# 18281818221/kalle-audio

Hardware: AMD Instinct MI355X
Metric: audio-seconds/sec (node) DiT train step, 10s@12.5Hz x1024 latents (higher is better)
Workload: dtype bf16; 1 GPU; DiT train step (fwd+bwd+allreduce+Adam), 24 blocks D=1536 h=24, 10 s @ 12.5 Hz x 1024 latents (T=125+1 prepend), S=130 x 768 cross-attn cond; DiT shape chosen by this build (reference defines none); global_batch=256, per_gpu_batch=256, parallelism=dp1, objective=v, io_channels=1024, global_cond_type=prepend

## Files before the change

### include/kalle_hip.h

```cpp
#ifndef KALLE_HIP_H
#define KALLE_HIP_H
#include <stdint.h>

#ifdef __cplusplus
extern "C" {
#endif

#define KALLE_BF16 0
#define KALLE_F32 1

int kalle_abi_version(void);
const char* kalle_target_arch(void);
const char* kalle_last_error(void);

typedef struct kalle_gemm_epilogue {
    const float* bias;
    const float* gate;
    int64_t ldg;
    int32_t rows_per_batch;
    const float* residual;
    int64_t ldr;
    int32_t accumulate;
    float alpha;
    int32_t c_rows_per_batch;
// ... 204 lines not shown
typedef struct kalle_opt_ctl {
    float   norm;
    float   coef;
    int32_t nonfinite;
    int32_t skip;
    int64_t skipped;
    int64_t clipped;
} kalle_opt_ctl;
int kalle_grad_norm_ws_bytes(int nslots);
int kalle_grad_sumsq(const float* grad, int64_t n, void* ws, int slot, int nslots, void* stream);
int kalle_grad_norm_finish(const void* ws, int nslots, float grad_scale, float max_norm, int skip_nonfinite,
                           kalle_opt_ctl* ctl, void* stream);
int kalle_adam_step_ctl(float* param, const float* grad, float* exp_avg, float* exp_avg_sq, void* param_bf16,
                        int64_t n, float lr, float beta1, float beta2, float eps, float weight_decay, int decoupled,
                        int step, float grad_scale, const kalle_opt_ctl* ctl, void* stream);

int kalle_weight_norm_fold(const float* v, const float* g, float* w_packed, int d0, int d1, int ksize,
                           int transposed, void* stream);
typedef struct kalle_act {
    int32_t code;
    int32_t logscale;
    const float* alpha;
    const float* beta;
    float param;
} kalle_act;
typedef struct kalle_conv_epilogue {
    const void* residual;
    float out_scale;
    int32_t accumulate;
    int32_t tanh;
// ... 159 lines not shown
```

### kalle_audio_amd/build.py

```python
import os
import subprocess
import sys
from concurrent.futures import ThreadPoolExecutor

HERE = os.path.dirname(os.path.abspath(__file__))
CSRC = os.path.join(HERE, "csrc")
OUT = os.path.join(HERE, "libkalle_hip.so")
SOURCES = ["gemm.hip", "gemm2.hip", "norm.hip", "elementwise.hip", "attention.hip", "conv1d.hip", "conv1d_bwd.hip",
           "llasa.hip", "conformer.hip"]
FLAGS = ["-O3", "--offload-arch=gfx950", "-fPIC", "-std=c++17", "-ffast-math", "-fno-finite-math-only",
         "-Wno-unused-value"]


def source_stamp():
    import hashlib
    h = hashlib.sha256()
    files = sorted(os.path.join(CSRC, f) for f in os.listdir(CSRC) if f.endswith((".hip", ".h")))
    files.append(os.path.join(HERE, "..", "include", "kalle_hip.h"))
    for f in files:
        h.update(os.path.basename(f).encode())
        h.update(open(f, "rb").read())
    return h.hexdigest()[:16]


def _needs(obj, deps):
    if not os.path.exists(obj):
        return True
    t = os.path.getmtime(obj)
    return any(os.path.getmtime(d) > t for d in deps)


def build(verbose=True, force=False, extra_flags=(), out=None, objdir_name="build", only=None):
    global OUT
    hipcc = os.environ.get("HIPCC", "/opt/rocm/bin/hipcc")
    objdir = os.path.join(HERE, objdir_name)
    out = out or OUT
    os.makedirs(objdir, exist_ok=True)
    hdrs = [os.path.join(CSRC, "common.h"), os.path.join(CSRC, "gemm_common.h"), os.path.join(HERE, "..", "include", "kalle_hip.h")]
    srcs = [s for s in SOURCES if os.path.exists(os.path.join(CSRC, s))]
    jobs = []
    for s in srcs:
        src = os.path.join(CSRC, s)
        obj = os.path.join(objdir, s.replace(".hip", ".o"))
        if force or _needs(obj, [src] + hdrs):
            jobs.append([hipcc] + FLAGS + list(extra_flags) + ["-c", src, "-o", obj])

    def run(cmd):
        if verbose:
            print(" ".join(cmd), flush=True)
        r = subprocess.run(cmd, capture_output=True, text=True)
        if r.returncode != 0:
            raise RuntimeError("hipcc failed:\n" + r.stdout + r.stderr)
        if verbose and r.stderr.strip():
# ... 18 lines not shown
```

### kalle_audio_amd/csrc/elementwise.hip

```cpp
#include <stdio.h>
#include <stdlib.h>

#include "common.h"
#include "../../include/kalle_hip.h"

namespace {

inline int grid_for(int64_t work_items, int block) {
    int64_t g = (work_items + block - 1) / block;
    if (g > 2048) g = 2048;
    if (g < 1) g = 1;
    return (int)g;
}

__global__ __launch_bounds__(256) void swiglu_fwd_kernel(const bf16_t* __restrict__ h, bf16_t* __restrict__ out,
                                                         int64_t rows, int inner) {
    const int cpr = inner >> 3;
    const int64_t total = rows * cpr;
    for (int64_t i = (int64_t)blockIdx.x * blockDim.x + threadIdx.x; i < total; i += (int64_t)gridDim.x * blockDim.x) {
        const int64_t r = i / cpr;
        const int c = (int)(i - r * cpr) * 8;
        const i32x4 xv = *reinterpret_cast<const i32x4*>(h + r * 2 * inner + c);
        const i32x4 gv = *reinterpret_cast<const i32x4*>(h + r * 2 * inner + inner + c);
        i32x4 o;
// ... 306 lines not shown
    const float wj = w[j];
    for (int b = 0; b < nbatch; ++b) {
        const float k = 6.283185307179586f * t[b];
        const float f = k * wj;
        acc += k * (dout[(int64_t)b * 2 * half + half + j] * cosf(f) - dout[(int64_t)b * 2 * half + j] * sinf(f));
    }
    dw[j] = acc;
}

__device__ __forceinline__ void adam_body(float* __restrict__ p, const float* __restrict__ g,
                                          float* __restrict__ m, float* __restrict__ v,
                                          bf16_t* __restrict__ pb, int64_t n, float lr, float b1, float b2,
                                          float eps, float wd, int decoupled, float bc1, float bc2,
                                          float gscale, const int64_t first, const int64_t stride) {
    const int64_t n4 = n >> 2;
    for (int64_t i = first; i < n4; i += stride) {
        f32x4 pv = reinterpret_cast<f32x4*>(p)[i];
        const f32x4 gv = reinterpret_cast<const f32x4*>(g)[i];
        f32x4 mv = reinterpret_cast<f32x4*>(m)[i];
        f32x4 vv = reinterpret_cast<f32x4*>(v)[i];
#pragma unroll
        for (int e = 0; e < 4; ++e) {
            float gr = gv[e] * gscale;
            if (decoupled) pv[e] *= (1.f - lr * wd); else gr += wd * pv[e];
            mv[e] = b1 * mv[e] + (1.f - b1) * gr;
            vv[e] = b2 * vv[e] + (1.f - b2) * gr * gr;
            const float denom = sqrtf(vv[e]) / bc2 + eps;
            pv[e] -= (lr / bc1) * (mv[e] / denom);
        }
        reinterpret_cast<f32x4*>(p)[i] = pv;
        reinterpret_cast<f32x4*>(m)[i] = mv;
        reinterpret_cast<f32x4*>(v)[i] = vv;
        if (pb) {
            i32x2 o;
            o[0] = (int)pack_bf16x2(pv[0], pv[1]);
            o[1] = (int)pack_bf16x2(pv[2], pv[3]);
            reinterpret_cast<i32x2*>(pb)[i] = o;
        }
    }
    if (blockIdx.x == 0 && threadIdx.x < (n & 3)) {
        const int64_t i = (n4 << 2) + threadIdx.x;
        float pv = p[i], gr = g[i] * gscale, mv = m[i], vv = v[i];
        if (decoupled) pv *= (1.f - lr * wd); else gr += wd * pv;
        mv = b1 * mv + (1.f - b1) * gr;
        vv = b2 * vv + (1.f - b2) * gr * gr;
        pv -= (lr / bc1) * (mv / (sqrtf(vv) / bc2 + eps));
        p[i] = pv; m[i] = mv; v[i] = vv;
        if (pb) pb[i] = f32_to_bf16(pv);
    }
}

__global__ __launch_bounds__(256) void adam_kernel(float* __restrict__ p, const float* __restrict__ g,
                                                   float* __restrict__ m, float* __restrict__ v,
                                                   bf16_t* __restrict__ pb, int64_t n, float lr, float b1, float b2,
                                                   float eps, float wd, int decoupled, float bc1, float bc2,
                                                   float gscale) {
    adam_body(p, g, m, v, pb, n, lr, b1, b2, eps, wd, decoupled, bc1, bc2, gscale,
              (int64_t)blockIdx.x * blockDim.x + threadIdx.x, (int64_t)gridDim.x * blockDim.x);
}

__global__ __launch_bounds__(256) void adam_ctl_kernel(float* __restrict__ p, const float* __restrict__ g,
                                                       float* __restrict__ m, float* __restrict__ v,
                                                       bf16_t* __restrict__ pb, int64_t n, float lr, float b1, float b2,
                                                       float eps, float wd, int decoupled, float bc1, float bc2,
                                                       float gscale, const kalle_opt_ctl* __restrict__ ctl) {
    if (ctl->skip) return;
    adam_body(p, g, m, v, pb, n, lr, b1, b2, eps, wd, decoupled, bc1, bc2, gscale * ctl->coef,
              (int64_t)blockIdx.x * blockDim.x + threadIdx.x, (int64_t)gridDim.x * blockDim.x);
}

__device__ __forceinline__ void sumsq_acc(const f32x4 x, double& acc, uint32_t& bad) {
#pragma unroll
    for (int e = 0; e < 4; ++e) {
        const float xe = x[e];
        const double d = (double)xe;
        acc += d * d;
        bad |= (uint32_t)((__builtin_bit_cast(uint32_t, xe) & 0x7f800000u) == 0x7f800000u);
    }
}

__global__ __launch_bounds__(KALLE_GRAD_NORM_BLOCK) void grad_sumsq_kernel(const float* __restrict__ g, int64_t n,
                                                                           double* __restrict__ part,
                                                                           int32_t* __restrict__ flag) {
// ... 225 lines not shown
}

extern "C" int kalle_adam_step_ctl(float* param, const float* grad, float* exp_avg, float* exp_avg_sq, void* param_bf16,
                                   int64_t n, float lr, float beta1, float beta2, float eps, float weight_decay,
                                   int decoupled, int step, float grad_scale, const kalle_opt_ctl* ctl, void* stream) {
    if (!param || !grad || !exp_avg || !exp_avg_sq || !ctl || n <= 0 || step <= 0) return KALLE_ERR_ARG;
    if ((uintptr_t)ctl & 7) return KALLE_ERR_ARG;
    const float bc1 = 1.f - powf(beta1, (float)step);
    const float bc2 = sqrtf(1.f - powf(beta2, (float)step));
    const int agrid = (int)std::min<int64_t>(((n >> 2) + 255) / 256 + 1, 16384);
    KALLE_LAUNCH(adam_ctl_kernel, dim3(agrid), dim3(256), 0, static_cast<hipStream_t>(stream), param,
                       grad, exp_avg, exp_avg_sq, static_cast<bf16_t*>(param_bf16), n, lr, beta1, beta2, eps,
                       weight_decay, decoupled, bc1, bc2, grad_scale, ctl);
    return kalle_check_launch();
}
extern "C" int kalle_grad_norm_ws_bytes(int nslots) {
    if (nslots <= 0 || nslots > (1 << 16)) return KALLE_ERR_ARG;
    return nslots * KALLE_GRAD_NORM_SLOT_BYTES;
}
extern "C" int kalle_grad_sumsq(const float* grad, int64_t n, void* ws, int slot, int nslots, void* stream) {
    if (!grad || !ws || n <= 0 || nslots <= 0 || nslots > (1 << 16) || slot < 0 || slot >= nslots) return KALLE_ERR_ARG;
    if (((uintptr_t)grad & 15) || ((uintptr_t)ws & 15)) return KALLE_ERR_ARG;
    char* base = static_cast<char*>(ws) + (int64_t)slot * KALLE_GRAD_NORM_SLOT_BYTES;
    KALLE_LAUNCH(grad_sumsq_kernel, dim3(KALLE_GRAD_NORM_PARTIALS), dim3(KALLE_GRAD_NORM_BLOCK), 0,
                 static_cast<hipStream_t>(stream), grad, n, reinterpret_cast<double*>(base),
                 reinterpret_cast<int32_t*>(base + KALLE_GRAD_NORM_PARTIALS * 8));
    return kalle_check_launch();
}
extern "C" int kalle_grad_norm_finish(const void* ws, int nslots, float grad_scale, float max_norm, int skip_nonfinite,
                                      kalle_opt_ctl* ctl, void* stream) {
// ... 45 lines not shown
```

### kalle_audio_amd/csrc/gemm2.hip

```cpp
#include <stdio.h>
#include <stdlib.h>
#include <string.h>

#include <algorithm>
#include <functional>
#include <type_traits>
#include <utility>

#include "gemm_common.h"
#include "../../include/kalle_hip.h"

namespace {

constexpr int BK2 = 64;
#define GPTR(p) ((const __attribute__((address_space(1))) void*)(p))

__device__ __attribute__((aligned(64))) const unsigned kalle_zero_block[16] = {0, 0, 0, 0, 0, 0, 0, 0, 0, 0, 0, 0, 0, 0, 0, 0};

template <bool KM, int R, int NW>
struct Loader {
    static constexpr int PER_WAVE = (R / 8) / NW;
    const bf16_t* src[PER_WAVE];
    int64_t kstep;

// ... 667 lines not shown
    hipDeviceProp_t prop;
    v = hipGetDeviceProperties(&prop, dev) == hipSuccess && prop.multiProcessorCount > 0 ? prop.multiProcessorCount : 256;
    v &= ~7;
    if (v < 8) v = 8;
    cached[dev & 63].store(v, std::memory_order_relaxed);
    return v;
}

#define MFMA32(FA, FB)                                                                                         \
    _Pragma("unroll") for (int mt = 0; mt < 8; ++mt) _Pragma("unroll") for (int nt = 0; nt < 4; ++nt)          \
        acc[mt][nt] = __builtin_amdgcn_mfma_f32_16x16x32_bf16(__builtin_bit_cast(bf16x8, FA[mt]),              \
                                                              __builtin_bit_cast(bf16x8, FB[nt]), acc[mt][nt], 0, 0, 0)

constexpr int SCHED_SETS = 256;
constexpr int SCHED_LINE = 32;
__device__ int kalle_gemm_sched[SCHED_SETS][9 * SCHED_LINE];

__device__ __forceinline__ int sched_issue(int* sched, int xcd) { return atomicAdd(sched + xcd * SCHED_LINE, 1); }
__device__ __forceinline__ int sched_resolve(int xcd, int raw, int first_round, int ntiles) {
    const int id = xcd + 8 * (first_round + raw);
    return id < ntiles ? id : ntiles;
}
__device__ __forceinline__ void sched_leave(int* sched, int nwg) {
    if (atomicAdd(sched + 8 * SCHED_LINE, 1) == nwg - 1) {
#pragma unroll
        for (int i = 0; i < 9; ++i) atomicExch(sched + i * SCHED_LINE, 0);
    }
}

template <bool A_KM, bool B_KM, bool C_F32, int GLU, bool XCD_RASTER, bool PERSIST>
__device__ __forceinline__ void gemm3_tiles(const GemmParams& p, int tile0, int tstride, int tile_end, int ntiles_raster, int kt0,
                                            int nk) {
    const int kvalid = p.K % BK2;
    const int tail_t = kvalid ? (p.K + BK2 - 1) / BK2 - 1 - kt0 : -1;
    constexpr int WN = 4, TM = 8, NW = 8;
    constexpr int BM = 256, BN = 256;
    constexpr int A_BYTES = BM * 128, B_BYTES = BN * 128, STAGE = A_BYTES + B_BYTES;
    extern __shared__ __attribute__((aligned(16))) char smem[];
    const unsigned lds0 = (unsigned)(size_t)LDS_PTR(char, smem);

    const int tid = threadIdx.x, lane = tid & 63;
// ... 143 lines not shown
                if (nk > 1) {
                    la.issue_at(smem + s_last, wave, lane, 1, tail_t, kvalid);
                    lb.issue_at(smem + s_last + A_BYTES, wave, lane, 1, tail_t, kvalid);
                }
                if (sched && tid == 0) drawn = sched_issue(sched, blockIdx.x & 7);
            }
        };
        wave_epilogue<C_F32, TM, GLU>(p, acc, smem + 2 * STAGE, wave, lane, m0 + arow, GLU == 1 ? tn * 128 + wn * 32 : n0 + bcol,
                                      hook, tile);
        prefetched = has_next;
        s0 = s_last ^ STAGE;
        if constexpr (!PERSIST) break;
    }
}

template <bool A_KM, bool B_KM, bool C_F32, int GLU = 0>
__global__ __launch_bounds__(512, 2) void gemm3_kernel(GemmParams p) {
    const int nk_all = (p.K + BK2 - 1) / BK2;
    const int ntiles = p.tiles_m * p.tiles_n;
    if constexpr (A_KM) {
        if (p.mix_na >= 0) {
            const int na = p.mix_na, sa = p.mix_sa;
            int bid = blockIdx.x, tile, slice, per;
            if (bid < na * sa) { tile = bid % na; slice = bid / na; per = (nk_all + sa - 1) / sa; }
            else { bid -= na * sa; const int nb = ntiles - na; tile = na + bid % nb; slice = bid / nb; per = (nk_all + sa) / (sa + 1); }
            const int kt0 = slice * per, nk = min(per, nk_all - kt0);
            if (nk <= 0) return;
            gemm3_tiles<A_KM, B_KM, C_F32, GLU, true, false>(p, tile, 0, tile + 1, ntiles, kt0, nk);
        } else {
            const int kt0 = blockIdx.y * p.ktiles_per_split;
            gemm3_tiles<A_KM, B_KM, C_F32, GLU, true, false>(p, blockIdx.x, 0, blockIdx.x + 1, ntiles, kt0,
                                                             min(p.ktiles_per_split, nk_all - kt0));
        }
    } else {
        gemm3_tiles<A_KM, B_KM, C_F32, GLU, true, true>(p, blockIdx.x, gridDim.x, ntiles, ntiles, 0, nk_all);
        if (p.sched_set > 0 && threadIdx.x == 0) sched_leave(&kalle_gemm_sched[p.sched_set - 1][0], gridDim.x);
    }
}

struct GroupProblem {
    const bf16_t* A;
    const bf16_t* B;
    float* C;
    int64_t lda, ldb, ldc;
    int M, N, K;
    int tiles_m, tiles_n, group_m;
    int unsplit, splits;
    int r1_start, r2_start;
};
struct GroupParams {
// ... 43 lines not shown
    p.alpha = 1.f;
    p.rows_per_batch = 1;
    p.accumulate = gp.overwrite ? 0 : 1;
    p.atomic = whole ? 0 : 1;
    const int ntiles = q.tiles_m * q.tiles_n, nk_all = (q.K + BK2 - 1) / BK2;
    p.tiles_m = q.tiles_m; p.tiles_n = q.tiles_n; p.group_m = q.group_m;
    int kt0 = 0, nk = nk_all;
    if (!whole) {
        const int per = (nk_all + q.splits - 1) / q.splits;
        kt0 = slice * per;
        nk = min(per, nk_all - kt0);
        if (nk <= 0) return;
    }
    gemm3_tiles<true, true, true, 0, false, false>(p, tile, 0, tile + 1, ntiles, kt0, nk);
}

template <bool A_KM, bool B_KM, bool C_F32, int GLU = 0>
int launch3(const GemmParams& p, hipStream_t st) {
    constexpr int lds = GEMM3_LDS;
    static std::atomic<uint64_t> lds_ok{0};
    kalle_allow_lds(reinterpret_cast<const void*>(gemm3_kernel<A_KM, B_KM, C_F32, GLU>), lds, lds_ok);
    dim3 grid(p.tiles_m * p.tiles_n, p.splits), block(512);
    if (p.mix_na >= 0) {
        const int ntiles = p.tiles_m * p.tiles_n;
        grid = dim3(p.mix_na * p.mix_sa + (ntiles - p.mix_na) * (p.mix_sa + 1), 1);
    } else if (!A_KM) {
        if (p.splits != 1) return KALLE_ERR_UNSUPPORTED;
        const int cus = kalle_cu_count();
        if ((int)grid.x > cus) {
            GemmParams q = p;
            grid.x = cus;
            static std::atomic<unsigned> next_set{0};
            hipStreamCaptureStatus cap = hipStreamCaptureStatusNone;
            const bool capturing = hipStreamIsCapturing(st, &cap) == hipSuccess && cap != hipStreamCaptureStatusNone;
            q.sched_set = !capturing ? 1 + (int)(next_set.fetch_add(1, std::memory_order_relaxed) % SCHED_SETS) : 0;
            KALLE_LAUNCH((gemm3_kernel<A_KM, B_KM, C_F32, GLU>), grid, block, lds, st, q);
            return kalle_check_launch();
        }
    }
    KALLE_LAUNCH((gemm3_kernel<A_KM, B_KM, C_F32, GLU>), grid, block, lds, st, p);
    return kalle_check_launch();
}

int launch3_layout(const GemmParams& p, bool a_km, bool b_km, bool f32, hipStream_t st) {
    if (!a_km && !b_km) return f32 ? launch3<false, false, true>(p, st) : launch3<false, false, false>(p, st);
    if (!a_km && b_km) return f32 ? launch3<false, true, true>(p, st) : launch3<false, true, false>(p, st);
    if (a_km && b_km) return launch3<true, true, true>(p, st);
    return KALLE_ERR_UNSUPPORTED;
}

// ... 348 lines not shown

namespace {
__global__ __launch_bounds__(256) void hold_cus_kernel(int ticks) {
    extern __shared__ char hold_smem[];
    if (ticks < 0) hold_smem[threadIdx.x] = 1;
    const unsigned long long t_end = __builtin_amdgcn_s_memrealtime() + (unsigned long long)ticks;
    while (__builtin_amdgcn_s_memrealtime() < t_end) __builtin_amdgcn_s_sleep(64);
}
}
extern "C" int kalle_debug_hold_cus(int nwg, int lds_bytes, int microseconds, void* stream) {
    if (nwg <= 0 || nwg > 4096 || lds_bytes < 0 || lds_bytes > 65536 || microseconds < 0 || microseconds > 1000000) return KALLE_ERR_ARG;
    KALLE_LAUNCH(hold_cus_kernel, dim3(nwg), dim3(256), lds_bytes, static_cast<hipStream_t>(stream), microseconds * 100);
    return kalle_check_launch();
}

static thread_local int g_last_plan = 0;
extern "C" int kalle_gemm_last_plan(void) { return g_last_plan; }

extern "C" int kalle_gemm_plan(const void* A, int64_t lda, int a_kmajor, const void* B, int64_t ldb, int b_kmajor,
                               void* C, int64_t ldc, int c_dtype, int M, int N, int K,
                               const kalle_gemm_epilogue* ep, int* plan) {
    if (!plan) return KALLE_ERR_ARG;
    GemmParams p; GemmPlan g;
    const int rc = plan_gemm(A, lda, a_kmajor, B, ldb, b_kmajor, C, ldc, c_dtype, M, N, K, ep, false, p, g);
    if (rc == KALLE_OK) *plan = g.word;
    return rc;
}

extern "C" int kalle_gemm_bf16(const void* A, int64_t lda, int a_kmajor, const void* B, int64_t ldb, int b_kmajor,
                               void* C, int64_t ldc, int c_dtype, int M, int N, int K,
// ... 145 lines not shown
```

### kalle_audio_amd/csrc/gemm_common.h

```cpp
#pragma once
#include "common.h"

struct GemmParams {
    const bf16_t* A;
    const bf16_t* B;
    void* C;
    int64_t lda, ldb, ldc;
    int M, N, K;
    const float* bias;
    const float* gate;
    int64_t ldg;
    int rows_per_batch;
    const float* residual;
    int64_t ldr;
    int accumulate;
    int tiles_n;
    float alpha;
    int c_rpb, c_brows, c_roff;
    const uint8_t* row_mask;
    int tiles_m, splits, ktiles_per_split, atomic, group_m, tile_n;
    int mix_na, mix_sa;
    int glu_mode, glu_inner;
    void* glu_aux;
    float* glu_dbias;
    int64_t slab_stride;
    unsigned long long* stamps;
    int sched_set;
};

__device__ __forceinline__ void gemm_tile_coords(int bid, int nwg, int tiles_m, int tiles_n, int gm, int& tm, int& tn) {
    const int qd = nwg >> 3, rm = nwg & 7, xcd = bid & 7;
    const int wg = (xcd < rm ? xcd * (qd + 1) : rm * (qd + 1) + (xcd - rm) * qd) + (bid >> 3);
    const int per_group = gm * tiles_n;
    const int group = wg / per_group;
    const int first_m = group * gm;
    const int gsz = min(gm, tiles_m - first_m);
    const int in = wg - group * per_group;
    tm = first_m + in % gsz;
    tn = in / gsz;
}

__device__ __forceinline__ int xcd_contiguous(int bid, int nwg) {
// ... 66 lines not shown
```

### kalle_audio_amd/engine.py

```python
import math
import contextlib
import os

import torch
import torch.distributed as dist

from . import ops


class FusedAdam(torch.optim.Optimizer):

    def __init__(self, params, lr=1e-3, betas=(0.9, 0.999), eps=1e-8, weight_decay=0.0, adam_w_mode=True):
        super().__init__(params, dict(lr=lr, betas=betas, eps=eps, weight_decay=weight_decay, adam_w_mode=adam_w_mode))

    @torch.no_grad()
    def step(self, closure=None):
        loss = closure() if closure is not None else None
        for g in self.param_groups:
            for p in g["params"]:
                if p.grad is None:
                    continue
                st = self.state[p]
                if not st:
                    st["step"] = 0
# ... 167 lines not shown
            self._norm_ws = ops.grad_norm_ws(len(self._norm_slot), device)
            self._ctl = ops.OptCtl(device)
        self.shard_opt = (os.environ.get("KALLE_SHARD_OPTIMIZER", "0") == "1" and comm_dtype == torch.float32
                          and self.world & (self.world - 1) == 0 and self.world <= 64)
        self._shard_bufs = {}
        self.overlap_adam = device.type == "cuda" and os.environ.get("KALLE_OVERLAP_ADAM", "1") != "0"
        side = self.overlap_adam or (device.type == "cuda" and self.shard_opt)
        self._opt_stream = torch.cuda.Stream(device=device) if side else None
        self._comm_stream = torch.cuda.Stream(device=device) if side else None
        self._comm_events = 0
        self._shard_ev = None
        self._opt_done = set()
        self._opt_lr = None
        self._overlap_now = False
        self.overlap_min_rows = int(os.environ.get("KALLE_OVERLAP_ADAM_MIN_ROWS", "4096"))
        for n, blk in self.blocks:
            pre = n + "."
            blk._kalle_grad_sinks = {k[len(pre):]: self.flat.grad_view(k) for k in self.flat.names if k.startswith(pre)}
            blk._kalle_grad_accumulate = False
            blk._kalle_bucket_key = pre if pre in self.flat.bucket_range else None
            blk._kalle_on_backward_done = self._on_block_done
        for (na, a), (nb, b_) in zip(self.blocks, self.blocks[1:]):
            if (isinstance(a, TransformerBlock) and isinstance(b_, TransformerBlock) and na.rsplit(".", 1)[0] == nb.rsplit(".", 1)[0]
                    and getattr(b_, "layer_ix", -1) == getattr(a, "layer_ix", -9) + 1):
                object.__setattr__(b_, "_kalle_prev_block", a)
        for n, p in named:
            if getattr(p, "_kalle_wants_sink", False) and bucket_of(n) == "_rest":
                p._kalle_grad_sink = self.flat.grad_view(n)

    def _comm_active(self):
# ... 146 lines not shown

    def _on_block_done(self, blk):
        key = blk._kalle_bucket_key
        if key is None or not self._boundary():
            return
        if self._sharded_active():
            ev = None
            if self.flat.grad.is_cuda:
                ev = torch.cuda.Event()
                ev.record(torch.cuda.current_stream())
            self._sharded_bucket(key, ev)
            return
        if not self._overlap_now:
            self._allreduce(self.flat.bucket_grad(key))
            return
        ev = torch.cuda.Event()
        ev.record(torch.cuda.current_stream())
        self._queue_bucket([key], ev)

    def _begin_optimizer_step(self):
        k = self.step_count + 1
        self._opt_lr = self.lr * (self.lr_schedule(k - 1) if self.lr_schedule else 1.0)
        self._opt_done = set()
        self._norm_done = set()
        self._norm_final = False
        self._comm_events = 0
        self._shard_ev = None

    def _adam_bucket(self, key):
        a, b = self.flat.bucket_range[key]
        self._adam_range(a, b)
        self._opt_done.add(key)

    def _adam_range(self, a, b, grad=None):
        if b <= a:
            return
        f = self.flat
        ops.adam_step(f.param[a:b], f.grad[a:b] if grad is None else grad, self.exp_avg[a:b], self.exp_avg_sq[a:b],
                      f.param_bf16[a:b] if f.param_bf16 is not None else None, lr=self._opt_lr, beta1=self.betas[0],
                      beta2=self.betas[1], eps=self.eps, weight_decay=self.weight_decay, decoupled=self.decoupled,
                      step=self.step_count + 1, grad_scale=1.0 / (self.world * self.grad_accum_steps))

    def _boundary(self):
        return (self.micro + 1) % self.grad_accum_steps == 0

    def _finish_comm(self):
        if self._overlap_now and self._boundary():
            cur = torch.cuda.current_stream()
            ev = torch.cuda.Event()
            ev.record(cur)
            done = self._norm_done if self._norm_gate else self._opt_done
            self._queue_bucket([k for k in self.flat.bucket_keys if k not in done], ev)
            if self._norm_on:
                with torch.cuda.stream(self._opt_stream):
                    self._norm_finish()
                    if self._norm_gate:
                        self._adam_ctl_all()
            timed = self.comm_timing is not None
            if timed:
                e0, e1 = torch.cuda.Event(enable_timing=True), torch.cuda.Event(enable_timing=True)
                e0.record()
# ... 47 lines not shown
        if first:
            if clear_once:
                self.flat.grad.zero_()
            else:
                if grouped:
                    for _, blk in self.blocks:
                        a, b = self.flat.small_range.get(blk._kalle_bucket_key, (0, 0))
                        if b > a:
                            self.flat.grad[a:b].zero_()
                for key in ("_rest", "_vae"):
                    if key in self.flat.bucket_range:
                        self.flat.bucket_grad(key).zero_()
        if self._boundary():
            self._begin_optimizer_step()
            self._overlap_now = self.overlap_adam and (rows >= self.overlap_min_rows or not self.blocks)
        loss.backward()
        self._finish_comm()
        if self._boundary():
            self.optimizer_step()
        self.micro += 1

    def enable_ema(self, **kw):
        self.ema_schedule = EMASchedule(**kw)
        self.ema = self.flat.param.clone()
        return self

    def _ema_update(self):
        d = self.ema_schedule.next()
        if d is None:
            return
# ... 92 lines not shown
```

### kalle_audio_amd/ops.py

```python
import ctypes
import os

import torch

from . import _lib
from ._lib import KALLE_BF16, KALLE_F32, GemmEpilogue, check


def _stream():
    return ctypes.c_void_p(torch.cuda.current_stream().cuda_stream)


def _dt(t):
    if t.dtype == torch.bfloat16:
        return KALLE_BF16
    if t.dtype == torch.float32:
        return KALLE_F32
    raise TypeError(f"unsupported dtype {t.dtype}")


def _p(t):
    if t is None:
        return None
    if not t.is_cuda:
# ... 359 lines not shown


WEIGHTS_EPOCH = 0


def adam_step(param, grad, exp_avg, exp_avg_sq, param_bf16, *, lr, beta1=0.9, beta2=0.999, eps=1e-8, weight_decay=0.0,
              decoupled=False, step=1, grad_scale=1.0):
    global WEIGHTS_EPOCH
    WEIGHTS_EPOCH += 1
    lib = _lib.load()
    check(lib.kalle_adam_step(_p(param), _p(grad), _p(exp_avg), _p(exp_avg_sq), _p(param_bf16), param.numel(), lr,
                              beta1, beta2, eps, weight_decay, int(decoupled), step, grad_scale, _stream()),
          "kalle_adam_step")


GRAD_NORM_PARTIALS = 1024
GRAD_NORM_BLOCK = 256
GRAD_NORM_UNROLL = 4


class OptCtl:

    def __init__(self, device):
        self.t = torch.zeros(8, device=device, dtype=torch.int32)
        self.norm = self.t[0:1].view(torch.float32)
        self.coef = self.t[1:2].view(torch.float32)
        self.nonfinite = self.t[2:3]
        self.skip = self.t[3:4]
        self.skipped = self.t[4:6].view(torch.int64)
        self.clipped = self.t[6:8].view(torch.int64)
# ... 638 lines not shown
```

Baseline: 11740 audio-seconds/sec.

## Run Adam bucket updates in GEMM tail workgroups via a device job ring

Adds a device-side ring of Adam jobs. During backward, each finished gradient bucket is appended to the ring instead of being queued on a separate optimizer stream. GEMM kernels get a variant that pulls Adam chunks from the ring, presumably in idle tail workgroups, and a flush kernel finishes any remaining chunks at the step boundary. The Adam math is also rewritten with FMAs and reciprocal approximations, and the ring path can use nontemporal loads and stores. The aim is to hide optimizer memory traffic under GEMM tails, at the cost of added atomics, extra GEMM register and LDS pressure, and slightly different rounding in Adam.

```diff
diff --git a/include/kalle_hip.h b/include/kalle_hip.h
--- a/include/kalle_hip.h
+++ b/include/kalle_hip.h
@@ -242,6 +242,20 @@
 int kalle_adam_step_ctl(float* param, const float* grad, float* exp_avg, float* exp_avg_sq, void* param_bf16,
                         int64_t n, float lr, float beta1, float beta2, float eps, float weight_decay, int decoupled,
                         int step, float grad_scale, const kalle_opt_ctl* ctl, void* stream);
+
+#define KALLE_ADAM_RING_JOBS 32
+#define KALLE_ADAM_CHUNK_FLOAT4 2048
+#define KALLE_ADAM_RING_QUERY_INTS (4 + 2 * KALLE_ADAM_RING_JOBS)
+int kalle_adam_ring_create(void** ring);
+int kalle_adam_ring_destroy(void* ring);
+int kalle_adam_ring_append(void* ring, float* param, const float* grad, float* exp_avg, float* exp_avg_sq, void* param_bf16,
+                           int64_t n, float lr, float beta1, float beta2, float eps, float weight_decay, int decoupled,
+                           int step, float grad_scale, int chunk_float4, void* stream);
+int kalle_adam_ring_pending(void* ring);
+int kalle_gemm_attach_adam_ring(void* ring);
+int kalle_adam_flush(void* ring, void* stream);
+int kalle_adam_ring_query(void* ring, int64_t* out, void* stream);
+int kalle_debug_adam_chunks(void* ring, int nwg, int threads, int lds_bytes, int take, void* stream);
 
 int kalle_weight_norm_fold(const float* v, const float* g, float* w_packed, int d0, int d1, int ksize,
                            int transposed, void* stream);
diff --git a/kalle_audio_amd/build.py b/kalle_audio_amd/build.py
--- a/kalle_audio_amd/build.py
+++ b/kalle_audio_amd/build.py
@@ -36,7 +36,8 @@
     objdir = os.path.join(HERE, objdir_name)
     out = out or OUT
     os.makedirs(objdir, exist_ok=True)
-    hdrs = [os.path.join(CSRC, "common.h"), os.path.join(CSRC, "gemm_common.h"), os.path.join(HERE, "..", "include", "kalle_hip.h")]
+    hdrs = [os.path.join(CSRC, "common.h"), os.path.join(CSRC, "gemm_common.h"), os.path.join(CSRC, "adam_tails.h"),
+            os.path.join(HERE, "..", "include", "kalle_hip.h")]
     srcs = [s for s in SOURCES if os.path.exists(os.path.join(CSRC, s))]
     jobs = []
     for s in srcs:
diff --git a/kalle_audio_amd/csrc/adam_tails.h b/kalle_audio_amd/csrc/adam_tails.h
--- /dev/null
+++ b/kalle_audio_amd/csrc/adam_tails.h
@@ -0,0 +1,157 @@
+#pragma once
+#include "common.h"
+
+constexpr int ADAM_RING_JOBS = 32;
+
+struct AdamScalars {
+    float lr, b1, b2, eps, wd, bc1, bc2, gscale;
+    int decoupled;
+};
+
+struct alignas(128) AdamJob {
+    float* p;
+    const float* g;
+    float* m;
+    float* v;
+    bf16_t* pb;
+    int64_t n;
+    AdamScalars s;
+    int chunk4;
+    int nt;
+    int nchunks;
+    alignas(128) int cursor;
+};
+
+struct alignas(128) AdamRing {
+    int njobs;
+    alignas(128) int head;
+    alignas(128) int64_t chunks_tails;
+    int64_t chunks_all;
+    AdamJob job[ADAM_RING_JOBS];
+};
+
+struct KalleAdamRing {
+    AdamRing* dev;
+    int njobs;
+};
+
+struct AdamConsts {
+    float wd, b1, b2, eps, gscale, lr, bc1;
+    float decay;
+    float inv_bc2;
+    int decoupled;
+};
+__device__ __forceinline__ AdamConsts adam_consts(float lr, float b1, float b2, float eps, float wd, int decoupled, float bc1,
+                                                  float bc2, float gscale) {
+    AdamConsts c;
+    c.wd = wd; c.b1 = b1; c.b2 = b2; c.eps = eps; c.gscale = gscale; c.lr = lr; c.bc1 = bc1;
+    c.decay = __builtin_fmaf(-lr, wd, 1.f);
+    c.inv_bc2 = __builtin_amdgcn_rcpf(bc2);
+    c.decoupled = decoupled;
+    return c;
+}
+__device__ __forceinline__ void adam_update(float& p, const float g, float& m, float& v, const AdamConsts& c) {
+#pragma clang fp reassociate(off) contract(off)
+    const float gs = g * c.gscale;
+    const float gr = c.decoupled ? gs : __builtin_fmaf(p, c.wd, gs);
+    const float pd = c.decoupled ? p * c.decay : p;
+    const float g2 = gr * gr;
+    v = __builtin_fmaf(__builtin_fmaf(-gr, gr, v), c.b2, g2);
+    m = __builtin_fmaf(m - gr, c.b1, gr);
+    const float denom = __builtin_fmaf(__builtin_amdgcn_sqrtf(v), c.inv_bc2, c.eps);
+    p = __builtin_fmaf(-(c.lr * m), __builtin_amdgcn_rcpf(c.bc1 * denom), pd);
+}
+__device__ __forceinline__ void adam_update4(f32x4& pv, const f32x4 gv, f32x4& mv, f32x4& vv, const AdamConsts& c) {
+#pragma unroll
+    for (int e = 0; e < 4; ++e) {
+        float p = pv[e], m = mv[e], v = vv[e];
+        adam_update(p, gv[e], m, v, c);
+        pv[e] = p; mv[e] = m; vv[e] = v;
+    }
+}
+__device__ __forceinline__ void adam_update1(float* __restrict__ p, const float* __restrict__ g, float* __restrict__ m,
+                                             float* __restrict__ v, bf16_t* __restrict__ pb, int64_t i, const AdamConsts& c) {
+    float pv = p[i], mv = m[i], vv = v[i];
+    adam_update(pv, g[i], mv, vv, c);
+    p[i] = pv; m[i] = mv; v[i] = vv;
+    if (pb) pb[i] = f32_to_bf16(pv);
+}
+
+constexpr int ADAM_CHUNK_UNROLL = 4;
+template <bool NT>
+__device__ __forceinline__ void adam_chunk(const AdamJob& job, int c) {
+    float* __restrict__ p = job.p;
+    const float* __restrict__ g = job.g;
+    float* __restrict__ m = job.m;
+    float* __restrict__ v = job.v;
+    bf16_t* __restrict__ pb = job.pb;
+    const AdamScalars s = job.s;
+    const AdamConsts k = adam_consts(s.lr, s.b1, s.b2, s.eps, s.wd, s.decoupled, s.bc1, s.bc2, s.gscale);
+    const int64_t n4 = job.n >> 2;
+    const int64_t begin = (int64_t)c * job.chunk4;
+    const int64_t end = min(begin + (int64_t)job.chunk4, n4);
+    const int nt = blockDim.x;
+    auto ld = [](const float* base, int64_t i) {
+        const f32x4* q = reinterpret_cast<const f32x4*>(base) + i;
+        return NT ? __builtin_nontemporal_load(q) : *q;
+    };
+    auto st = [](float* base, int64_t i, const f32x4 x) {
+        f32x4* q = reinterpret_cast<f32x4*>(base) + i;
+        if (NT) __builtin_nontemporal_store(x, q); else *q = x;
+    };
+    for (int64_t i0 = begin + threadIdx.x; i0 < end; i0 += (int64_t)ADAM_CHUNK_UNROLL * nt) {
+        f32x4 pv[ADAM_CHUNK_UNROLL], gv[ADAM_CHUNK_UNROLL], mv[ADAM_CHUNK_UNROLL], vv[ADAM_CHUNK_UNROLL];
+#pragma unroll
+        for (int u = 0; u < ADAM_CHUNK_UNROLL; ++u) {
+            const int64_t i = i0 + (int64_t)u * nt;
+            if (i < end) { pv[u] = ld(p, i); gv[u] = ld(g, i); mv[u] = ld(m, i); vv[u] = ld(v, i); }
+        }
+#pragma unroll
+        for (int u = 0; u < ADAM_CHUNK_UNROLL; ++u) {
+            const int64_t i = i0 + (int64_t)u * nt;
+            if (i < end) {
+                adam_update4(pv[u], gv[u], mv[u], vv[u], k);
+                st(p, i, pv[u]); st(m, i, mv[u]); st(v, i, vv[u]);
+                if (pb) {
+                    i32x2 o;
+                    o[0] = (int)pack_bf16x2(pv[u][0], pv[u][1]);
+                    o[1] = (int)pack_bf16x2(pv[u][2], pv[u][3]);
+                    i32x2* q = reinterpret_cast<i32x2*>(pb) + i;
+                    if (NT) __builtin_nontemporal_store(o, q); else *q = o;
+                }
+            }
+        }
+    }
+    if (c == job.nchunks - 1 && (int)threadIdx.x < (int)(job.n & 3))
+        adam_update1(p, g, m, v, pb, (n4 << 2) + threadIdx.x, k);
+}
+
+__device__ __forceinline__ void adam_chunks(AdamRing* ring, volatile int* box, int* stop, int stop_at, int take) {
+    int j = 0, njobs = 0;
+    if (threadIdx.x == 0) {
+        njobs = min(__hip_atomic_load(&ring->njobs, __ATOMIC_RELAXED, __HIP_MEMORY_SCOPE_AGENT), ADAM_RING_JOBS);
+        j = njobs > 0 ? min(atomicAdd(&ring->head, 0), njobs) : 0;
+    }
+    for (int it = 0;; it ^= 2) {
+        if (threadIdx.x == 0) {
+            int c = -1;
+            if (!stop || atomicAdd(stop, 0) < stop_at) {
+                while (j < njobs) {
+                    c = atomicAdd(&ring->job[j].cursor, take);
+                    if (c < ring->job[j].nchunks) break;
+                    c = -1;
+                    atomicMax(&ring->head, ++j);
+                }
+            }
+            box[it] = j;
+            box[it + 1] = c;
+        }
+        __syncthreads();
+        const int jj = box[it], c = box[it + 1];
+        if (c < 0) break;
+        const AdamJob& job = ring->job[jj];
+        const int cend = min(c + take, job.nchunks);
+        if (job.nt) { for (int k = c; k < cend; ++k) adam_chunk<true>(job, k); }
+        else { for (int k = c; k < cend; ++k) adam_chunk<false>(job, k); }
+    }
+}
diff --git a/kalle_audio_amd/csrc/elementwise.hip b/kalle_audio_amd/csrc/elementwise.hip
--- a/kalle_audio_amd/csrc/elementwise.hip
+++ b/kalle_audio_amd/csrc/elementwise.hip
@@ -2,6 +2,7 @@
 #include <stdlib.h>
 
 #include "common.h"
+#include "adam_tails.h"
 #include "../../include/kalle_hip.h"
 
 namespace {
@@ -344,20 +345,13 @@
                                           float eps, float wd, int decoupled, float bc1, float bc2,
                                           float gscale, const int64_t first, const int64_t stride) {
     const int64_t n4 = n >> 2;
+    const AdamConsts k = adam_consts(lr, b1, b2, eps, wd, decoupled, bc1, bc2, gscale);
     for (int64_t i = first; i < n4; i += stride) {
         f32x4 pv = reinterpret_cast<f32x4*>(p)[i];
         const f32x4 gv = reinterpret_cast<const f32x4*>(g)[i];
         f32x4 mv = reinterpret_cast<f32x4*>(m)[i];
         f32x4 vv = reinterpret_cast<f32x4*>(v)[i];
-#pragma unroll
-        for (int e = 0; e < 4; ++e) {
-            float gr = gv[e] * gscale;
-            if (decoupled) pv[e] *= (1.f - lr * wd); else gr += wd * pv[e];
-            mv[e] = b1 * mv[e] + (1.f - b1) * gr;
-            vv[e] = b2 * vv[e] + (1.f - b2) * gr * gr;
-            const float denom = sqrtf(vv[e]) / bc2 + eps;
-            pv[e] -= (lr / bc1) * (mv[e] / denom);
-        }
+        adam_update4(pv, gv, mv, vv, k);
         reinterpret_cast<f32x4*>(p)[i] = pv;
         reinterpret_cast<f32x4*>(m)[i] = mv;
         reinterpret_cast<f32x4*>(v)[i] = vv;
@@ -369,14 +363,7 @@
         }
     }
     if (blockIdx.x == 0 && threadIdx.x < (n & 3)) {
-        const int64_t i = (n4 << 2) + threadIdx.x;
-        float pv = p[i], gr = g[i] * gscale, mv = m[i], vv = v[i];
-        if (decoupled) pv *= (1.f - lr * wd); else gr += wd * pv;
-        mv = b1 * mv + (1.f - b1) * gr;
-        vv = b2 * vv + (1.f - b2) * gr * gr;
-        pv -= (lr / bc1) * (mv / (sqrtf(vv) / bc2 + eps));
-        p[i] = pv; m[i] = mv; v[i] = vv;
-        if (pb) pb[i] = f32_to_bf16(pv);
+        adam_update1(p, g, m, v, pb, (n4 << 2) + threadIdx.x, k);
     }
 }
 
@@ -397,6 +384,37 @@
     if (ctl->skip) return;
     adam_body(p, g, m, v, pb, n, lr, b1, b2, eps, wd, decoupled, bc1, bc2, gscale * ctl->coef,
               (int64_t)blockIdx.x * blockDim.x + threadIdx.x, (int64_t)gridDim.x * blockDim.x);
+}
+
+__global__ void adam_ring_append_kernel(AdamRing* ring, AdamJob job) {
+    const int j = ring->njobs;
+    if (j >= ADAM_RING_JOBS) return;
+    job.cursor = 0;
+    ring->job[j] = job;
+    __threadfence();
+    ring->njobs = j + 1;
+}
+__global__ void adam_ring_account_kernel(AdamRing* ring) {
+    int64_t took = 0, all = 0;
+    for (int j = 0; j < ring->njobs; ++j) {
+        took += min(atomicAdd(&ring->job[j].cursor, 0), ring->job[j].nchunks);
+        all += ring->job[j].nchunks;
+    }
+    ring->chunks_tails += took;
+    ring->chunks_all += all;
+}
+constexpr int ADAM_FLUSH_TAKE = 4, ADAM_FLUSH_GRID = 2048, ADAM_FLUSH_BLOCK = 512;
+__global__ __launch_bounds__(ADAM_FLUSH_BLOCK) void adam_flush_kernel(AdamRing* ring) {
+    __shared__ int box[4];
+    adam_chunks(ring, box, nullptr, 0, ADAM_FLUSH_TAKE);
+}
+__global__ __launch_bounds__(512) void adam_probe_kernel(AdamRing* ring, int take) {
+    extern __shared__ __attribute__((aligned(16))) char probe_smem[];
+    adam_chunks(ring, reinterpret_cast<volatile int*>(probe_smem), nullptr, 0, take);
+}
+__global__ void adam_ring_reset_kernel(AdamRing* ring) {
+    if (threadIdx.x < ADAM_RING_JOBS) atomicExch(&ring->job[threadIdx.x].cursor, 0);
+    if (threadIdx.x == 0) { atomicExch(&ring->head, 0); ring->njobs = 0; }
 }
 
 __device__ __forceinline__ void sumsq_acc(const f32x4 x, double& acc, uint32_t& bad) {
@@ -652,6 +670,94 @@
                        weight_decay, decoupled, bc1, bc2, grad_scale, ctl);
     return kalle_check_launch();
 }
+static_assert(ADAM_RING_JOBS == KALLE_ADAM_RING_JOBS, "the ring of adam_tails.h and the header's constant");
+static bool adam_tails_nt() {
+    static const bool nt = [] { const char* e = getenv("KALLE_ADAM_TAILS_NT"); return !(e && e[0] == '0'); }();
+    return nt;
+}
+extern "C" int kalle_adam_ring_create(void** ring) {
+    if (!ring) return KALLE_ERR_ARG;
+    *ring = nullptr;
+    AdamRing* dev = nullptr;
+    if (hipMalloc(reinterpret_cast<void**>(&dev), sizeof(AdamRing)) != hipSuccess) return KALLE_ERR_LAUNCH;
+    if (hipMemset(dev, 0, sizeof(AdamRing)) != hipSuccess) { (void)hipFree(dev); return KALLE_ERR_LAUNCH; }
+    *ring = new KalleAdamRing{dev, 0};
+    return KALLE_OK;
+}
+extern "C" int kalle_adam_ring_destroy(void* ring) {
+    if (!ring) return KALLE_ERR_ARG;
+    KalleAdamRing* r = static_cast<KalleAdamRing*>(ring);
+    const bool ok = hipFree(r->dev) == hipSuccess;
+    delete r;
+    return ok ? KALLE_OK : KALLE_ERR_LAUNCH;
+}
+extern "C" int kalle_adam_ring_append(void* ring, float* param, const float* grad, float* exp_avg, float* exp_avg_sq,
+                                      void* param_bf16, int64_t n, float lr, float beta1, float beta2, float eps,
+                                      float weight_decay, int decoupled, int step, float grad_scale, int chunk_float4,
+                                      void* stream) {
+    if (!ring || !param || !grad || !exp_avg || !exp_avg_sq || n <= 0 || step <= 0 || chunk_float4 < 0) return KALLE_ERR_ARG;
+    if (((uintptr_t)param | (uintptr_t)grad | (uintptr_t)exp_avg | (uintptr_t)exp_avg_sq) & 15) return KALLE_ERR_ARG;
+    if ((uintptr_t)param_bf16 & 7) return KALLE_ERR_ARG;
+    KalleAdamRing* r = static_cast<KalleAdamRing*>(ring);
+    if (r->njobs >= ADAM_RING_JOBS) return KALLE_ERR_UNSUPPORTED;
+    AdamJob job{};
+    job.p = param; job.g = grad; job.m = exp_avg; job.v = exp_avg_sq; job.pb = static_cast<bf16_t*>(param_bf16);
+    job.n = n;
+    job.s.lr = lr; job.s.b1 = beta1; job.s.b2 = beta2; job.s.eps = eps; job.s.wd = weight_decay;
+    job.s.bc1 = 1.f - powf(beta1, (float)step);
+    job.s.bc2 = sqrtf(1.f - powf(beta2, (float)step));
+    job.s.gscale = grad_scale;
+    job.s.decoupled = decoupled;
+    job.nt = adam_tails_nt() ? 1 : 0;
+    job.chunk4 = chunk_float4 > 0 ? chunk_float4 : KALLE_ADAM_CHUNK_FLOAT4;
+    const int64_t nchunks = std::max<int64_t>(((n >> 2) + job.chunk4 - 1) / job.chunk4, 1);
+    if (nchunks > (1 << 30)) return KALLE_ERR_ARG;
+    job.nchunks = (int)nchunks;
+    KALLE_LAUNCH(adam_ring_append_kernel, dim3(1), dim3(1), 0, static_cast<hipStream_t>(stream), r->dev, job);
+    const int rc = kalle_check_launch();
+    if (rc == KALLE_OK) ++r->njobs;
+    return rc;
+}
+extern "C" int kalle_adam_ring_pending(void* ring) {
+    return ring ? static_cast<KalleAdamRing*>(ring)->njobs : KALLE_ERR_ARG;
+}
+extern "C" int kalle_adam_flush(void* ring, void* stream) {
+    if (!ring) return KALLE_ERR_ARG;
+    KalleAdamRing* r = static_cast<KalleAdamRing*>(ring);
+    if (r->njobs == 0) return KALLE_OK;
+    hipStream_t st = static_cast<hipStream_t>(stream);
+    KALLE_LAUNCH(adam_ring_account_kernel, dim3(1), dim3(1), 0, st, r->dev);
+    KALLE_LAUNCH(adam_flush_kernel, dim3(ADAM_FLUSH_GRID), dim3(ADAM_FLUSH_BLOCK), 0, st, r->dev);
+    KALLE_LAUNCH(adam_ring_reset_kernel, dim3(1), dim3(64), 0, st, r->dev);
+    r->njobs = 0;
+    return kalle_check_launch();
+}
+extern "C" int kalle_debug_adam_chunks(void* ring, int nwg, int threads, int lds_bytes, int take, void* stream) {
+    if (!ring || nwg <= 0 || nwg > 65536 || threads < 64 || threads > 512 || (threads & 63) || take < 1 || take > 64)
+        return KALLE_ERR_ARG;
+    if (lds_bytes < 16 || lds_bytes > 160 * 1024) return KALLE_ERR_ARG;
+    const int lds = lds_bytes;
+    static std::atomic<uint64_t> lds_ok{0};
+    kalle_allow_lds(reinterpret_cast<const void*>(adam_probe_kernel), 160 * 1024, lds_ok);
+    KALLE_LAUNCH(adam_probe_kernel, dim3(nwg), dim3(threads), lds, static_cast<hipStream_t>(stream),
+                 static_cast<KalleAdamRing*>(ring)->dev, take);
+    return kalle_check_launch();
+}
+extern "C" int kalle_adam_ring_query(void* ring, int64_t* out, void* stream) {
+    if (!ring || !out) return KALLE_ERR_ARG;
+    KalleAdamRing* r = static_cast<KalleAdamRing*>(ring);
+    hipStream_t st = static_cast<hipStream_t>(stream);
+    static AdamRing host;
+    if (hipMemcpyAsync(&host, r->dev, sizeof(AdamRing), hipMemcpyDeviceToHost, st) != hipSuccess) return KALLE_ERR_LAUNCH;
+    if (hipStreamSynchronize(st) != hipSuccess) return KALLE_ERR_LAUNCH;
+    out[0] = host.njobs; out[1] = host.chunks_tails; out[2] = host.chunks_all; out[3] = 0;
+    for (int j = 0; j < ADAM_RING_JOBS; ++j) {
+        const bool live = j < host.njobs;
+        out[4 + 2 * j] = live ? std::min(host.job[j].cursor, host.job[j].nchunks) : 0;
+        out[5 + 2 * j] = live ? host.job[j].nchunks : 0;
+    }
+    return KALLE_OK;
+}
 extern "C" int kalle_grad_norm_ws_bytes(int nslots) {
     if (nslots <= 0 || nslots > (1 << 16)) return KALLE_ERR_ARG;
     return nslots * KALLE_GRAD_NORM_SLOT_BYTES;
diff --git a/kalle_audio_amd/csrc/gemm2.hip b/kalle_audio_amd/csrc/gemm2.hip
--- a/kalle_audio_amd/csrc/gemm2.hip
+++ b/kalle_audio_amd/csrc/gemm2.hip
@@ -8,6 +8,7 @@
 #include <utility>
 
 #include "gemm_common.h"
+#include "adam_tails.h"
 #include "../../include/kalle_hip.h"
 
 namespace {
@@ -705,7 +706,7 @@
 
 constexpr int SCHED_SETS = 256;
 constexpr int SCHED_LINE = 32;
-__device__ int kalle_gemm_sched[SCHED_SETS][9 * SCHED_LINE];
+__device__ int kalle_gemm_sched[SCHED_SETS][10 * SCHED_LINE];
 
 __device__ __forceinline__ int sched_issue(int* sched, int xcd) { return atomicAdd(sched + xcd * SCHED_LINE, 1); }
 __device__ __forceinline__ int sched_resolve(int xcd, int raw, int first_round, int ntiles) {
@@ -715,7 +716,7 @@
 __device__ __forceinline__ void sched_leave(int* sched, int nwg) {
     if (atomicAdd(sched + 8 * SCHED_LINE, 1) == nwg - 1) {
 #pragma unroll
-        for (int i = 0; i < 9; ++i) atomicExch(sched + i * SCHED_LINE, 0);
+        for (int i = 0; i < 10; ++i) atomicExch(sched + i * SCHED_LINE, 0);
     }
 }
 
@@ -889,7 +890,12 @@
     }
 }
 
-template <bool A_KM, bool B_KM, bool C_F32, int GLU = 0>
+__device__ __forceinline__ void adam_tail(AdamRing* ring, int* out_of_tiles) {
+    extern __shared__ __attribute__((aligned(16))) char smem[];
+    if (threadIdx.x == 0) atomicAdd(out_of_tiles, 1);
+    adam_chunks(ring, reinterpret_cast<volatile int*>(smem + 2 * (256 + 256) * 128), out_of_tiles, (int)gridDim.x, 1);
+}
+template <bool A_KM, bool B_KM, bool C_F32, int GLU = 0, bool TAILS = false>
 __global__ __launch_bounds__(512, 2) void gemm3_kernel(GemmParams p) {
     const int nk_all = (p.K + BK2 - 1) / BK2;
     const int ntiles = p.tiles_m * p.tiles_n;
@@ -909,6 +915,9 @@
         }
     } else {
         gemm3_tiles<A_KM, B_KM, C_F32, GLU, true, true>(p, blockIdx.x, gridDim.x, ntiles, ntiles, 0, nk_all);
+        if constexpr (TAILS) {
+            if (p.sched_set > 0 && p.adam_ring) adam_tail(p.adam_ring, &kalle_gemm_sched[p.sched_set - 1][9 * SCHED_LINE]);
+        }
         if (p.sched_set > 0 && threadIdx.x == 0) sched_leave(&kalle_gemm_sched[p.sched_set - 1][0], gridDim.x);
     }
 }
@@ -982,6 +991,8 @@
     }
     gemm3_tiles<true, true, true, 0, false, false>(p, tile, 0, tile + 1, ntiles, kt0, nk);
 }
+
+std::atomic<AdamRing*> g_adam_ring{nullptr};
 
 template <bool A_KM, bool B_KM, bool C_F32, int GLU = 0>
 int launch3(const GemmParams& p, hipStream_t st) {
@@ -1002,6 +1013,13 @@
             hipStreamCaptureStatus cap = hipStreamCaptureStatusNone;
             const bool capturing = hipStreamIsCapturing(st, &cap) == hipSuccess && cap != hipStreamCaptureStatusNone;
             q.sched_set = !capturing ? 1 + (int)(next_set.fetch_add(1, std::memory_order_relaxed) % SCHED_SETS) : 0;
+            q.adam_ring = !capturing ? g_adam_ring.load(std::memory_order_relaxed) : nullptr;
+            if (q.adam_ring) {
+                static std::atomic<uint64_t> lds_ok_t{0};
+                kalle_allow_lds(reinterpret_cast<const void*>(gemm3_kernel<A_KM, B_KM, C_F32, GLU, true>), lds, lds_ok_t);
+                KALLE_LAUNCH((gemm3_kernel<A_KM, B_KM, C_F32, GLU, true>), grid, block, lds, st, q);
+                return kalle_check_launch();
+            }
             KALLE_LAUNCH((gemm3_kernel<A_KM, B_KM, C_F32, GLU>), grid, block, lds, st, q);
             return kalle_check_launch();
         }
@@ -1380,6 +1398,11 @@
     return kalle_check_launch();
 }
 
+extern "C" int kalle_gemm_attach_adam_ring(void* ring) {
+    g_adam_ring.store(ring ? static_cast<KalleAdamRing*>(ring)->dev : nullptr, std::memory_order_relaxed);
+    return KALLE_OK;
+}
+
 static thread_local int g_last_plan = 0;
 extern "C" int kalle_gemm_last_plan(void) { return g_last_plan; }
 
diff --git a/kalle_audio_amd/csrc/gemm_common.h b/kalle_audio_amd/csrc/gemm_common.h
--- a/kalle_audio_amd/csrc/gemm_common.h
+++ b/kalle_audio_amd/csrc/gemm_common.h
@@ -26,6 +26,7 @@
     int64_t slab_stride;
     unsigned long long* stamps;
     int sched_set;
+    struct AdamRing* adam_ring;
 };
 
 __device__ __forceinline__ void gemm_tile_coords(int bid, int nwg, int tiles_m, int tiles_n, int gm, int& tm, int& tn) {
diff --git a/kalle_audio_amd/engine.py b/kalle_audio_amd/engine.py
--- a/kalle_audio_amd/engine.py
+++ b/kalle_audio_amd/engine.py
@@ -205,6 +205,13 @@
         self._opt_lr = None
         self._overlap_now = False
         self.overlap_min_rows = int(os.environ.get("KALLE_OVERLAP_ADAM_MIN_ROWS", "4096"))
+        self.adam_tails = self.overlap_adam and os.environ.get("KALLE_ADAM_TAILS", "1") != "0"
+        self.tails_min_rows = int(os.environ.get("KALLE_ADAM_TAILS_MIN_ROWS", "4096"))
+        self._ring = None
+        self.tails_chunk = int(os.environ.get("KALLE_ADAM_TAILS_CHUNK", "0"))
+        self._tails_now = False
+        self._opt_stream_used = False
+        self.tails_steps = 0
         for n, blk in self.blocks:
             pre = n + "."
             blk._kalle_grad_sinks = {k[len(pre):]: self.flat.grad_view(k) for k in self.flat.names if k.startswith(pre)}
@@ -381,8 +388,11 @@
         if not self._overlap_now:
             self._allreduce(self.flat.bucket_grad(key))
             return
+        if self._tails_now and self._tails_append(key):
+            return
         ev = torch.cuda.Event()
         ev.record(torch.cuda.current_stream())
+        self._opt_stream_used = True
         self._queue_bucket([key], ev)
 
     def _begin_optimizer_step(self):
@@ -394,6 +404,25 @@
         self._comm_events = 0
         self._shard_ev = None
 
+    def _tails_append(self, key):
+        if self._ring is None:
+            self._ring = ops.AdamRing()
+        ring = self._ring
+        if ring.full():
+            return False
+        a, b = self.flat.bucket_range[key]
+        if b > a:
+            f = self.flat
+            ring.append(f.param[a:b], f.grad[a:b], self.exp_avg[a:b], self.exp_avg_sq[a:b],
+                        f.param_bf16[a:b] if f.param_bf16 is not None else None, lr=self._opt_lr, beta1=self.betas[0],
+                        beta2=self.betas[1], eps=self.eps, weight_decay=self.weight_decay, decoupled=self.decoupled,
+                        step=self.step_count + 1, grad_scale=1.0 / (self.world * self.grad_accum_steps),
+                        chunk_float4=self.tails_chunk)
+            if ops.AdamRing._attached is not ring:
+                ring.attach()
+        self._opt_done.add(key)
+        return True
+
     def _adam_bucket(self, key):
         a, b = self.flat.bucket_range[key]
         self._adam_range(a, b)
@@ -411,7 +440,26 @@
     def _boundary(self):
         return (self.micro + 1) % self.grad_accum_steps == 0
 
+    def _tails_flush(self):
+        ring = self._ring
+        if ops.AdamRing._attached is ring:
+            ops.AdamRing.detach()
+        timed = self.comm_timing is not None
+        if timed:
+            e0, e1 = torch.cuda.Event(enable_timing=True), torch.cuda.Event(enable_timing=True)
+            e0.record()
+        if ring.pending():
+            self.tails_steps += 1
+        ring.flush()
+        if timed:
+            e1.record()
+            self.comm_timing.append((e0, e1, 0))
+
     def _finish_comm(self):
+        if self._tails_now and self._boundary() and self._ring is not None:
+            self._tails_flush()
+            if not self._opt_stream_used:
+                return
         if self._overlap_now and self._boundary():
             cur = torch.cuda.current_stream()
             ev = torch.cuda.Event()
@@ -489,6 +537,10 @@
         if self._boundary():
             self._begin_optimizer_step()
             self._overlap_now = self.overlap_adam and (rows >= self.overlap_min_rows or not self.blocks)
+            self._tails_now = (self._overlap_now and self.adam_tails and rows >= self.tails_min_rows and self.world == 1
+                               and not self._comm_active() and not self._sharded_active() and not self._norm_on
+                               and not torch.cuda.is_current_stream_capturing())
+            self._opt_stream_used = False
         loss.backward()
         self._finish_comm()
         if self._boundary():
diff --git a/kalle_audio_amd/ops.py b/kalle_audio_amd/ops.py
--- a/kalle_audio_amd/ops.py
+++ b/kalle_audio_amd/ops.py
@@ -397,6 +397,76 @@
           "kalle_adam_step")
 
 
+ADAM_RING_JOBS = 32
+ADAM_CHUNK_FLOAT4 = 2048
+
+
+class AdamRing:
+
+    def __init__(self):
+        self._lib = _lib.load()
+        h = ctypes.c_void_p()
+        check(self._lib.kalle_adam_ring_create(ctypes.byref(h)), "kalle_adam_ring_create")
+        self._h = h
+        self._keep = []
+
+    def pending(self):
+        return self._lib.kalle_adam_ring_pending(self._h)
+
+    def full(self):
+        return self.pending() >= ADAM_RING_JOBS
+
+    def append(self, param, grad, exp_avg, exp_avg_sq, param_bf16, *, lr, beta1=0.9, beta2=0.999, eps=1e-8,
+               weight_decay=0.0, decoupled=False, step=1, grad_scale=1.0, chunk_float4=0):
+        global WEIGHTS_EPOCH
+        WEIGHTS_EPOCH += 1
+        for t in (param, grad, exp_avg, exp_avg_sq):
+            assert t.dtype == torch.float32 and t.is_contiguous() and t.numel() == param.numel()
+        assert param_bf16 is None or (param_bf16.dtype == torch.bfloat16 and param_bf16.is_contiguous()
+                                      and param_bf16.numel() == param.numel())
+        check(self._lib.kalle_adam_ring_append(self._h, _p(param), _p(grad), _p(exp_avg), _p(exp_avg_sq), _p(param_bf16),
+                                               param.numel(), lr, beta1, beta2, eps, weight_decay, int(decoupled), step,
+                                               grad_scale, int(chunk_float4), _stream()), "kalle_adam_ring_append")
+        self._keep.append((param, grad, exp_avg, exp_avg_sq, param_bf16))
+
+    _attached = None
+
+    def attach(self):
+        check(self._lib.kalle_gemm_attach_adam_ring(self._h), "kalle_gemm_attach_adam_ring")
+        AdamRing._attached = self
+
+    @staticmethod
+    def detach():
+        check(_lib.load().kalle_gemm_attach_adam_ring(None), "kalle_gemm_attach_adam_ring")
+        AdamRing._attached = None
+
+    def flush(self):
+        check(self._lib.kalle_adam_flush(self._h, _stream()), "kalle_adam_flush")
+        self._keep = []
+
+    def query(self):
+        out = (ctypes.c_int64 * (4 + 2 * ADAM_RING_JOBS))()
+        check(self._lib.kalle_adam_ring_query(self._h, out, _stream()), "kalle_adam_ring_query")
+        return {"jobs": [(out[4 + 2 * j], out[5 + 2 * j]) for j in range(out[0])], "tails": out[1], "all": out[2]}
+
+    def close(self):
+        if self._h:
+            if self.pending() > 0:
+                self.flush()
+            if AdamRing._attached is self:
+                AdamRing.detach()
+            h, self._h = self._h, None
+            check(self._lib.kalle_adam_ring_destroy(h), "kalle_adam_ring_destroy")
+
+    def __del__(self):
+        import sys
+        if getattr(self, "_h", None) and not sys.is_finalizing():
+            try:
+                self.close()
+            except Exception:
+                pass
+
+
 GRAD_NORM_PARTIALS = 1024
 GRAD_NORM_BLOCK = 256
 GRAD_NORM_UNROLL = 4
```

After: 11850 audio-seconds/sec, median of 6. No clear change (+0.9%).
